# johnviljoen/f16_mpc_oop_py

Hardware: AMD Instinct MI355X
Metric: F16 env steps/sec (hifi Nguyen model, explicit Euler dt=1ms, batch 4096 per GPU) (higher is better)
Workload: dtype f64

## Files before the change

### f16_mpc_oop_py_amd/csrc/f16_dynamics.hip

```cpp
#include <hip/hip_runtime.h>
#include <stdlib.h>

#include <type_traits>

#include "../../include/f16_hip.h"
#include "f16_ctx.h"
#include "f16_plant.hpp"
#include "f16_rollout_common.hpp"
#include "f16_plant_quad.hpp"
#include "f16_mppi.hpp"
#include "f16_gain_sched.hpp"

namespace f16 {

struct CostArgs : SchedArgs {
  const double *x0;
  const double *x_ref;
  const double *u_ref;
  double *x_end;
  long B0, ld0;
  f16_cost_weights w;
};
struct GainSchedArgs : SchedArgs {
  f16_gain_grid grid;
// ... 484 lines not shown
        aero_part<3>((const double *)tab, xa, a.flags, o, sa);
      } else if (wave == 1) {
        aero_part<1>((const double *)tab, xa, a.flags, o, sa);
      } else if (wave == 2) {
        aero_part<2>((const double *)tab, xa, a.flags, o, sa);
      } else {
        double vt = xa[6];
        if (vt <= 0.01) vt = 0.01;
        double mach, qbar, ps;
        atmos_dev(xa[2], vt, mach, qbar, ps);
        xt[12][lane] = qbar; xt[13][lane] = ps;
        aero_part<4>((const double *)tab, xa, a.flags, o, sa);
        if (live) {
          double xq[18];
#pragma unroll
          for (int k = 0; k < 17; ++k) xq[k] = xa[k];
          xq[17] = x[17];
          if (LQR) {
            const double e0 = kq[9] - xa[9], e1 = kq[10] - xa[10], e2 = kq[11] - xa[11];
            double uc[4] = {u[0], 0, 0, 0};
#pragma unroll
            for (int i = 0; i < 3; ++i) ul[i] = uc[1 + i] = lqr_action(kq[3 * i], kq[3 * i + 1], kq[3 * i + 2], e0, e1, e2, u[1 + i]);
            actuators_dev(xq, uc, qbar, ps, xd);
          } else
          actuators_dev(xq, u, qbar, ps, xd);
#pragma unroll
          for (int k = 12; k < 18; ++k) x[k] += xd[k] * a.dt;
        }
        if (tr && --until_store == 0) {
          until_store = a.traj_every;
          if (valid) {
#pragma unroll
            for (int k = 12; k < 18; ++k) __builtin_nontemporal_store(x[k], tr + k * a.ld);
          }
          tr += 18 * a.ld;
        }
        if constexpr (SCHED) if (newrow) {
          ra.take(a, NR, LQR ? kq + 9 : u, a.out + b);
          if (LQR) { ul[0] = u[1]; ul[1] = u[2]; ul[2] = u[3]; }
        }
      }
      const int slot = wave == 1 ? 0 : (wave == 0 ? 3 : (wave == 2 ? 6 : 9));
      xt[slot][lane] = o[0]; xt[slot + 1][lane] = o[1]; xt[slot + 2][lane] = o[2];
      xst[wave][lane] = sa;
      STAMP(tB)
      __syncthreads();
      STAMP(tC)
      if (wave == 0 || wave == 2) {
        double ls[3], ldm[3], ts[3], td[3];
#pragma unroll
        for (int k = 0; k < 3; ++k) { ls[k] = xt[k][lane]; ldm[k] = xt[3 + k][lane]; ts[k] = xt[6 + k][lane]; td[k] = xt[9 + k][lane]; }
        Totals tt;
        compose_totals(ls, ldm, ts, td, a.xcg, tt);
        if (wave == 0) {
          if (live) {
            p.qbar = xt[12][lane]; p.ps = xt[13][lane];
            st |= xst[0][lane] | xst[1][lane] | xst[2][lane] | xst[3][lane];
            plant_forces(xa, p, tt.Cx, tt.Cy, tt.Cz, xd);
#pragma unroll
            for (int k = 0; k < 9; ++k) x[k] += xd[k] * a.dt;
          }
        } else {
          if (live) {
            plant_moments(x[9], x[10], x[11], xt[12][lane], tt.Cl, tt.Cm, tt.Cn, xd);
#pragma unroll
            for (int k = 9; k < 12; ++k) x[k] += xd[k] * a.dt;
          }
          if (tr && --until_store == 0) {
            until_store = a.traj_every;
            if (valid) {
#pragma unroll
              for (int k = 9; k < 12; ++k) __builtin_nontemporal_store(x[k], tr + k * a.ld);
            }
            tr += 18 * a.ld;
          }
        }
      }
    }
#ifdef F16_EXP_STAMP4W
    if (lane == 0 && blockIdx.x == 0 && a.traj) {
      double *d = a.traj + 18 * a.ld * 2 + wave * 4;
      d[0] = (double)tD; d[1] = (double)tA; d[2] = (double)tB; d[3] = (double)tC;
    }
#endif
    if (valid && wave != 1) {
      bool finite = true;
      const int k0 = wave == 0 ? 0 : (wave == 2 ? 9 : 12), k1 = wave == 0 ? 9 : (wave == 2 ? 12 : 18);
#pragma unroll
      for (int k = 0; k < 18; ++k)
        if (k >= k0 && k < k1) { finite = finite && isfinite(x[k]); a.out[k * a.ld + b] = x[k]; }
      if (st & ST_ENVELOPE) st |= envelope_state_bits(x) & (((1 << k1) - (1 << k0)) << 8);
      if (a.status) atomicOr(&a.status[b], st | (finite ? 0 : ST_NONFINITE));
      if (LQR && wave == 3 && a.u_out) {
        a.u_out[b] = u[0];
#pragma unroll
        for (int i = 0; i < 3; ++i) a.u_out[(1 + i) * a.ld + b] = ul[i];
      }
    }
    __syncthreads();
  }
}

template <int GROUPS, bool LQR = false, bool SCHED = false>
__global__ __launch_bounds__(256 * GROUPS) void k_rollout_q(RolloutArgs<SCHED> a) {
  constexpr int NA = 16 * GROUPS;
  constexpr bool G1 = GROUPS == 1;
  __shared__ __attribute__((aligned(16))) double tab[TABLE_IMAGE_DOUBLES];
  __shared__ double xs[18][NA], xt[11][NA];
  __shared__ int xenv[3][NA], xst[2][NA];
  __shared__ double xpsi[3][NA];
#ifdef F16_EXP_STAMPQ
  const unsigned long long tstage0 = __builtin_amdgcn_s_memtime();
#endif
  {
    const double2 *src = reinterpret_cast<const double2 *>(a.tab);
    double2 *dst = reinterpret_cast<double2 *>(tab);
    for (int i = threadIdx.x; i < TABLE_IMAGE_DOUBLES / 2; i += 256 * GROUPS) dst[i] = src[i];
    __syncthreads();
  }
#ifdef F16_EXP_STAMPQ
  const unsigned long long tstage = __builtin_amdgcn_s_memtime() - tstage0;
#endif
  const int role = G1 ? __builtin_amdgcn_readfirstlane((threadIdx.x >> 6) & 3) : (threadIdx.x >> 6) & 3;
  const int grp = threadIdx.x >> 8, lane = threadIdx.x & 63, ac = 16 * grp + (lane >> 2), s = lane & 3;
  const bool envchk = !(a.flags & FLAG_NO_ENVELOPE);
  for (long b0 = (long)blockIdx.x * NA; b0 < a.B; b0 += (long)gridDim.x * NA) {
    const bool valid = b0 + ac < a.B;
    const long b = valid ? b0 + ac : a.B - 1;
    double x[18];
#pragma unroll
    for (int k = 0; k < 18; ++k) x[k] = a.out[k * a.ld + b];
    double ucmd = a.u[s * a.ld + b];
    double kr0 = 0, kr1 = 0, kr2 = 0, dm0 = 0, dm1 = 0, dm2 = 0, ulast = ucmd;
    if (LQR && role == 3) {
      const long row = 9 * (s > 0 ? s - 1 : 0) + 4;
      kr0 = a.K[row * a.ld + b]; kr1 = a.K[(row + 1) * a.ld + b]; kr2 = a.K[(row + 2) * a.ld + b];
      dm0 = a.dem[b]; dm1 = a.dem[a.ld + b]; dm2 = a.dem[2 * a.ld + b];
    }
    double xact = s == 0 ? x[12] : (s == 1 ? x[13] : (s == 2 ? x[14] : x[15]));
    int st = a.status ? a.status[b] : 0;
    double *tr = a.traj ? a.traj + b : nullptr;
    int until_store = a.traj_every;
    QuadCell qc = quad_cell_none();
    LongCorners klong = {};
    LatCorners klat = {};
    RowAhead<1, false> ra;
    double dmq = 0;
    const int rs = LQR && s == 3 ? 2 : s;
    if constexpr (SCHED) {
      dmq = s == 0 ? dm0 : (s == 1 ? dm1 : dm2);
      ra.init(a, LQR ? 3 : 4, a.out + b, rs * a.ld, role == 3);
      ra.settle();
    }
    if (G1 && role == 0 && s == 0) {
      double sp, cp;
      F16_SINCOS_K(reloaded(QUAD_K.sc), x[5], &sp, &cp);
      xpsi[1][ac] = sp; xpsi[2][ac] = cp;
    }
#ifdef F16_EXP_STAMPQ
    unsigned long long tA = 0, tB = 0, tC = 0, tD = 0, t0 = __builtin_amdgcn_s_memtime();
#if F16_EXP_STAMPQ + 0 == 2
#define QSTAMP_WAIT 0xC07F
#else
#define QSTAMP_WAIT 0
#endif
#define QSTAMP(acc) { __builtin_amdgcn_s_waitcnt(QSTAMP_WAIT); unsigned long long t1 = __builtin_amdgcn_s_memtime(); acc += t1 - t0; t0 = t1; }
    unsigned long long tK = 0, tk0 = 0;
#define QK_BEGIN { __builtin_amdgcn_s_waitcnt(QSTAMP_WAIT); tk0 = __builtin_amdgcn_s_memtime(); }
#define QK_END { __builtin_amdgcn_s_waitcnt(QSTAMP_WAIT); tK += __builtin_amdgcn_s_memtime() - tk0; }
#else
#define QSTAMP(acc)
#define QK_BEGIN
#define QK_END
#endif
    if constexpr (G1) {
      switch (role) {
        case 0: {
          constexpr int wave = 0;
#include "f16_quad_steps.inc"
        } break;
        case 1: {
          constexpr int wave = 1;
#include "f16_quad_steps.inc"
        } break;
        case 2: {
          constexpr int wave = 2;
#include "f16_quad_steps.inc"
        } break;
        default: {
          constexpr int wave = 3;
#include "f16_quad_steps.inc"
        } break;
      }
    } else {
      const int wave = role;
#include "f16_quad_steps.inc"
    }
#ifdef F16_EXP_STAMPQ
    if (lane == 0 && blockIdx.x == 0 && a.traj) {
      double *d = a.traj + 18 * a.ld * 2 + role * 4;
      d[0] = (double)tD; d[1] = (double)tA; d[2] = (double)tB; d[3] = (double)tC;
      a.traj[18 * a.ld * 2 + a.ld + role] = (double)tstage;
      a.traj[18 * a.ld * 2 + a.ld + 4 + role] = (double)tK;
    }
#endif
    if (valid) {
      if (role == 2 && s == 0) {
        bool finite = true;
#pragma unroll
        for (int k = 0; k < 9; ++k) { finite = finite && isfinite(x[k]); a.out[k * a.ld + b] = x[k]; }
        if (st & ST_ENVELOPE) st |= envelope_state_bits(x) & (0x1FF << 8);
        if (a.status) atomicOr(&a.status[b], st | (finite ? 0 : ST_NONFINITE));
      } else if (role == 1 && s == 0) {
        bool finite = true;
#pragma unroll
        for (int k = 9; k < 12; ++k) { finite = finite && isfinite(x[k]); a.out[k * a.ld + b] = x[k]; }
        if (st & ST_ENVELOPE) st |= envelope_state_bits(x) & (0x7 << 17);
        if (a.status) atomicOr(&a.status[b], st | (finite ? 0 : ST_NONFINITE));
      } else if (role == 3) {
        a.out[(12 + s) * a.ld + b] = xact;
        bool finite = isfinite(xact);
        if (s < 2) { const double v = s == 0 ? x[16] : x[17]; finite = finite && isfinite(v); a.out[(16 + s) * a.ld + b] = v; }
        if (st & ST_ENVELOPE) {
          const double lim = s == 1 ? 25.0 : (s == 2 ? 21.5 : 30.0);
          if (s == 0 ? (xact < 1000 || xact > 19000) : (xact < -lim || xact > lim)) st |= 1 << (8 + 12 + s);
          if (s == 0 && (x[16] < 0. || x[16] > 25)) st |= 1 << (8 + 16);
        }
        if (a.status) atomicOr(&a.status[b], st | (finite ? 0 : ST_NONFINITE));
        if (LQR && a.u_out) a.u_out[s * a.ld + b] = ulast;
      }
    }
    __syncthreads();
  }
}

struct LinArgsL {
  double *x;
  const double *Ad, *Bd, *K, *xref, *u0;
  double *trx, *tru;
  long B, ld;
  int nsteps, every;
  unsigned track;
};
__global__ __launch_bounds__(64, 1) void k_rollout_lqr_linear(LinArgsL a) {
  const long b = (long)blockIdx.x * 64 + threadIdx.x;
  if (b >= a.B) return;
  double A[81], Bm[27], K[27], x[9], xr[9], u0[3];
#pragma unroll
  for (int e = 0; e < 81; ++e) A[e] = a.Ad[e * a.ld + b];
#pragma unroll
  for (int e = 0; e < 27; ++e) { Bm[e] = a.Bd[e * a.ld + b]; K[e] = a.K[e * a.ld + b]; }
#pragma unroll
  for (int j = 0; j < 9; ++j) { x[j] = a.x[j * a.ld + b]; xr[j] = a.xref[j * a.ld + b]; }
#pragma unroll
  for (int c = 0; c < 3; ++c) u0[c] = a.u0 ? a.u0[c * a.ld + b] : 0.0;
  double *px = a.trx ? a.trx + b : nullptr, *pu = a.tru ? a.tru + b : nullptr;
  int until = a.every;
  for (int t = 0; t < a.nsteps; ++t) {
    double e[9], u[3], xn[9];
#pragma unroll
    for (int j = 0; j < 9; ++j) e[j] = (((a.track >> j) & 1u) ? xr[j] : x[j]) - x[j];
#pragma unroll
    for (int c = 0; c < 3; ++c) {
      double s = 0.0;
#pragma unroll
      for (int j = 0; j < 9; ++j) s += K[9 * c + j] * e[j];
      u[c] = -s + u0[c];
    }
#pragma unroll
    for (int r = 0; r < 9; ++r) {
      double s = 0.0, v = 0.0;
#pragma unroll
      for (int j = 0; j < 9; ++j) s += A[9 * r + j] * x[j];
#pragma unroll
      for (int c = 0; c < 3; ++c) v += Bm[3 * r + c] * u[c];
      xn[r] = s + v;
    }
#pragma unroll
    for (int r = 0; r < 9; ++r) x[r] = xn[r];
    if (--until == 0) {
      until = a.every;
      if (px) {
#pragma unroll
        for (int r = 0; r < 9; ++r) __builtin_nontemporal_store(x[r], px + r * a.ld);
        px += 9 * a.ld;
      }
      if (pu) {
#pragma unroll
        for (int c = 0; c < 3; ++c) __builtin_nontemporal_store(u[c], pu + c * a.ld);
        pu += 3 * a.ld;
      }
    }
  }
#pragma unroll
  for (int r = 0; r < 9; ++r) a.x[r * a.ld + b] = x[r];
}

template <int BLOCK>
__global__ __launch_bounds__(BLOCK) void k_xdot_na(DynArgs a) {
  __shared__ __attribute__((aligned(16))) double tab[TABLE_IMAGE_DOUBLES];
  if (a.fi == 1) stage_tables(tab, a.tab);
  for (long b = (long)blockIdx.x * BLOCK + threadIdx.x; b < a.B; b += (long)gridDim.x * BLOCK) {
    double sv[18], xd9[9];
#pragma unroll
    for (int k = 0; k < 18; ++k) sv[k] = a.x[k * a.ld + b];
    sv[3] = a.u[0 * a.ld + b]; sv[4] = a.u[1 * a.ld + b]; sv[7] = a.u[2 * a.ld + b]; sv[8] = a.u[3 * a.ld + b];
    sv[9] = a.u[4 * a.ld + b]; sv[10] = a.u[5 * a.ld + b]; sv[11] = a.u[6 * a.ld + b];
    sv[17] = a.u[7 * a.ld + b]; sv[16] = a.u[8 * a.ld + b];
    sv[13] = a.u3[0 * a.ld + b]; sv[14] = a.u3[1 * a.ld + b]; sv[15] = a.u3[2 * a.ld + b];
    int st = 0;
    calc_xdot_na((const double *)tab, a.lofi, sv, xd9, a.xcg, a.fi, a.flags, st);
#pragma unroll
    for (int k = 0; k < 9; ++k) a.out[k * a.ld + b] = xd9[k];
    if (a.status) a.status[b] |= st;
  }
}

}

using namespace f16;


extern "C" int f16_xdot_batch(f16_ctx *ctx, const double *x, const double *u, double *xdot, int32_t *status, long B,
                              long ld, double xcg, int fi_flag, unsigned flags, void *stream) {
  if (int rc = check_common(ctx, x, xdot, B, ld)) return rc;
  if (!u) return set_error(F16_EINVAL, "u is NULL");
  if (B == 0) return F16_OK;
  DynArgs a = base_args<DynArgs>(ctx, B, ld, xcg, fi_flag, flags, status);
  a.x = x; a.u = u; a.out = xdot;
  const Geometry g = geometry(B, fi_flag);
  by_block(g, [&](auto block) {
    constexpr int BLOCK = decltype(block)::value;
    if (fi_flag == 0) hipLaunchKernelGGL((k_xdot<BLOCK, 0>), dim3(g.grid), dim3(BLOCK), 0, (hipStream_t)stream, a);
    else hipLaunchKernelGGL((k_xdot<BLOCK, -1>), dim3(g.grid), dim3(BLOCK), 0, (hipStream_t)stream, a);
  });
  return hip_check(hipGetLastError(), "f16_xdot_batch launch");
}

extern "C" int f16_nlplant_batch(f16_ctx *ctx, const double *xu, double *xdot, int32_t *status, long B, long ld,
                                 double xcg, int fi_flag, unsigned flags, void *stream) {
  if (int rc = check_common(ctx, xu, xdot, B, ld)) return rc;
  if (B == 0) return F16_OK;
  DynArgs a = base_args<DynArgs>(ctx, B, ld, xcg, fi_flag, flags, status);
  a.x = xu; a.out = xdot;
  if (B <= 256) {
    hipLaunchKernelGGL((k_nlplant<64, false>), dim3((unsigned)((B + 63) / 64)), dim3(64), 0, (hipStream_t)stream, a);
  } else {
    const Geometry g = geometry(B, fi_flag);
    by_block(g, [&](auto block) {
      constexpr int BLOCK = decltype(block)::value;
      hipLaunchKernelGGL((k_nlplant<BLOCK, true>), dim3(g.grid), dim3(BLOCK), 0, (hipStream_t)stream, a);
    });
  }
  return hip_check(hipGetLastError(), "f16_nlplant_batch launch");
}

// ... 298 lines not shown
```

### f16_mpc_oop_py_amd/csrc/f16_plant.hpp

```cpp
#pragma once
#include <hip/hip_runtime.h>

#include "f16_tables.h"

namespace f16 {

constexpr int ST_ALPHA1 = 1, ST_ALPHA2 = 2, ST_BETA = 4, ST_EL = 8, ST_ENVELOPE = 16, ST_NONFINITE = 32;
constexpr unsigned FLAG_FIX_CLR = 1u, FLAG_NO_ENVELOPE = 2u, FLAG_NO_CELL_CACHE = 16u;

#define F16_DEV __device__ __forceinline__

#ifdef F16_FAST_DIV
#define F16_DIVC(x, c) ((x) * (1.0 / (c)))
#else
#define F16_DIVC(x, c) ((x) / (c))
#endif

__device__ __forceinline__ double f16_rcp(double x) {
#ifdef F16_FAST_DIV
  double r = __builtin_amdgcn_rcp(x);
  r = fma(r, fma(-x, r, 1.0), r);
  r = fma(r, fma(-x, r, 1.0), r);
  return r;
#else
  return 1.0 / x;
#endif
}

struct Axis {
  int j;
  double l;
  double m;
};

F16_DEV double lerp(double f1, double f2, const Axis &a) { return a.l * f2 + a.m * f1; }

F16_DEV double fma_vvs(double a, double b, double c) {
  double d;
  asm("v_fma_f64 %0, %1, %2, %3" : "=v"(d) : "v"(a), "v"(b), "s"(c));
  return d;
}
F16_DEV double fma_svv(double a, double b, double c) {
  double d;
  asm("v_fma_f64 %0, %1, %2, %3" : "=v"(d) : "s"(a), "v"(b), "v"(c));
  return d;
}

struct PowK {
  double log2e, ln2_hi, ln2_lo, nln2_hi, nln2_lo, two_thirds;
  double E[10];
  double L[7];
};
constexpr PowK POW_K = {
    1.44269504088896338700e+00, 6.93147180559945286227e-01, 2.31904681384629955842e-17, -6.93147180559945286227e-01,
    -2.31904681384629955842e-17, 6.66666666666666629659e-01,
    {2.50223225676461415e-08, 2.76309034901126543e-07, 2.75575145458253105e-06, 2.48014910390950412e-05, 1.98412695891155217e-04,
     1.38888889459163820e-03, 8.33333333345504315e-03, 4.16666666665197541e-02, 1.66666666666664770e-01, 5.00000000000001221e-01},
    {1.53670161652585818e-01, 1.52503063567000663e-01, 1.81863527724766383e-01, 2.22221384831011309e-01, 2.85714293974435540e-01,
     3.99999999961319630e-01, 6.66666666666728247e-01}};

F16_DEV double log_k(const PowK &K, double x) {
  const double m = __builtin_amdgcn_frexp_mant(x);
  const bool lo = m < K.two_thirds;
  const double sc = lo ? 2.0 : 1.0;
  const int e = __builtin_amdgcn_frexp_exp(x) + (lo ? -1 : 0);
  const double ym1 = fma(m, sc, -1.0), yp1 = fma(m, sc, 1.0);
  const double ylo = fma(m, sc, -(yp1 + -1.0));
  double r = __builtin_amdgcn_rcp(yp1);
  r = fma(fma(-yp1, r, 1.0), r, r);
  r = fma(fma(-yp1, r, 1.0), r, r);
  const double q = ym1 * r;
  const double p = yp1 * q;
  const double pl = fma(q, ylo, fma(q, yp1, -p));
  const double s25 = fma(yp1, q, pl);
  const double s27 = pl - fma(-yp1, q, s25);
  const double d28 = ym1 - s25;
  const double d32 = d28 + (((ym1 - d28) - s25) - s27);
  const double h = fma(r, d32, q);
  const double l = fma(r, d32, -fma(-ym1, r, h));
  const double z = h * h;
  double c = fma_vvs(z, K.L[0], K.L[1]);
#pragma unroll
  for (int k = 2; k < 7; ++k) c = fma_vvs(z, c, K.L[k]);
  const double a44 = __builtin_ldexp(h, 1), a45 = __builtin_ldexp(l, 1);
  const double t46 = h * z;
  const double u48 = fma(t46, c, a44);
  const double u50 = fma(t46, c, -(u48 - a44));
  const double u51 = a45 + u50;
  const double u52 = u48 + u51;
  const double u54 = u51 - (u52 - u48);
  const double f = (double)e;
  const double g56n = f * K.nln2_hi;
  const double g59 = fma_svv(K.ln2_lo, f, fma_svv(K.ln2_hi, f, g56n));
  const double g60 = fma_svv(K.ln2_hi, f, g59);
  const double g62 = g59 - fma_svv(K.nln2_hi, f, g60);
  const double w63 = g60 + u52;
  const double w64 = w63 - g60;
  const double w68 = (u52 - w64) + (g60 - (w63 - w64));
  const double v69 = g62 + u54;
  const double v70 = v69 - g62;
  const double v74 = (u54 - v70) + (g62 - (v69 - v70));
  const double k75 = v69 + w68;
  const double k76 = w63 + k75;
  const double k80 = k76 + (v74 + (k75 - (k76 - w63)));
  double res = __builtin_fabs(x) == __builtin_inf() ? x : k80;
  res = x < 0.0 ? __builtin_nan("") : res;
  return x == 0.0 ? -__builtin_inf() : res;
}

F16_DEV double exp_k(const PowK &K, double x) {
  const double n = rint(x * K.log2e);
  const double r = fma_svv(K.nln2_lo, n, fma_svv(K.nln2_hi, n, x));
  double c = fma_vvs(r, K.E[0], K.E[1]);
#pragma unroll
  for (int k = 2; k < 10; ++k) c = fma_vvs(r, c, K.E[k]);
  c = fma(r, c, 1.0);
  c = fma(r, c, 1.0);
  double res = __builtin_ldexp(c, (int)n);
  res = x > 1024.0 ? __builtin_inf() : res;
  return x < -1075.0 ? 0.0 : res;
}

template <typename PW>
F16_DEV void atmos_with(double alt, double vt, double &mach, double &qbar, double &ps, PW pw) {
  const double rho0 = 2.377e-3;
  const double tfac = 1 - .703e-5 * alt;
  double temp = 519.0 * tfac;
  if (alt >= 35000.0) temp = 390;
#ifdef F16_FAST_POW
  const double t2 = tfac * tfac;
  const double rho = rho0 * ((t2 * t2) * pw(tfac));
#else
  const double rho = rho0 * pow(tfac, 4.14);
#endif
  mach = vt / sqrt(1.4 * 1716.3 * temp);
  qbar = .5 * rho * (vt * vt);
  ps = 1715.0 * rho * temp;
  if (ps == 0) ps = 1715;
}
F16_DEV void atmos_dev(double alt, double vt, double &mach, double &qbar, double &ps) {
  atmos_with(alt, vt, mach, qbar, ps, [](double tfac) { return exp(0.14 * log(tfac)); });
}
F16_DEV void atmos_dev_k(const PowK &K, double alt, double vt, double &mach, double &qbar, double &ps) {
  atmos_with(alt, vt, mach, qbar, ps, [&K](double tfac) { return exp_k(K, 0.14 * log_k(K, tfac)); });
}


struct SinCosK {
  double two_over_pi, npio2[3];
  double S[8], C[9];
};
constexpr SinCosK SINCOS_K = {
    6.36619772367581382433e-01, {-1.57079632673412561417e+00, -6.07710050630396597660e-11, -2.02226624879595063154e-21},
    {-1.66666666666666657e-01, 8.33333333333333322e-03, -1.98412698412698413e-04, 2.75573192239858925e-06, -2.50521083854417202e-08, 1.60590438368216133e-10, -7.64716373181981641e-13, 2.81145725434552060e-15},
    {-5.00000000000000000e-01, 4.16666666666666644e-02, -1.38888888888888894e-03, 2.48015873015873016e-05, -2.75573192239858883e-07, 2.08767569878681002e-09, -1.14707455977297245e-11, 4.77947733238738525e-14, -1.56192069685862253e-16}};

struct QuadK { SinCosK sc; PowK pw; };
static __constant__ const QuadK QUAD_K = {SINCOS_K, POW_K};
template <typename T>
F16_DEV T reloaded(const T &t) {
  static_assert(sizeof(T) % sizeof(double) == 0, "a table of doubles");
  unsigned long p = reinterpret_cast<unsigned long>(&t);
  asm volatile("" : "+s"(p));
  const __attribute__((address_space(4))) double *q = (const __attribute__((address_space(4))) double *)p;
  T k;
  double *d = reinterpret_cast<double *>(&k);
#pragma unroll
  for (unsigned i = 0; i < sizeof(T) / sizeof(double); ++i) d[i] = q[i];
  return k;
}

#ifdef F16_FAST_TRIG
F16_DEV void sincos_quadrant(double n, double s0, double c0, double *sn, double *cs) {
  const int k = (int)n & 3;
  const double a = (k & 1) ? c0 : s0, b = (k & 1) ? s0 : c0;
  *sn = (k & 2) ? -a : a;
  *cs = ((k + 1) & 2) ? -b : b;
}

F16_DEV void sincos_bf(double x, double *sn, double *cs) {
  constexpr SinCosK K = SINCOS_K;
  const double n = rint(x * K.two_over_pi);
  double r = fma(-n, -K.npio2[0], x);
  r = fma(-n, -K.npio2[1], r);
  r = fma(-n, -K.npio2[2], r);
  const double z = r * r;
  double p = K.S[7], q = K.C[8];
#pragma unroll
  for (int k = 6; k >= 0; --k) p = fma(p, z, K.S[k]);
#pragma unroll
  for (int k = 7; k >= 0; --k) q = fma(q, z, K.C[k]);
  const double s0 = fma(r * z, p, r), c0 = fma(z, q, 1.0);
  sincos_quadrant(n, s0, c0, sn, cs);
}

F16_DEV void sincos_bf_k(const SinCosK &K, double x, double *sn, double *cs) {
  const double n = rint(x * K.two_over_pi);
  double r = fma_svv(K.npio2[0], n, x);
  r = fma_svv(K.npio2[1], n, r);
  r = fma_svv(K.npio2[2], n, r);
  const double z = r * r;
  double p = K.S[7], q = K.C[8];
#pragma unroll
  for (int k = 6; k >= 0; --k) p = fma_vvs(p, z, K.S[k]);
#pragma unroll
  for (int k = 7; k >= 0; --k) q = fma_vvs(q, z, K.C[k]);
  const double s0 = fma(r * z, p, r), c0 = fma(z, q, 1.0);
  sincos_quadrant(n, s0, c0, sn, cs);
}
#define F16_SINCOS(x, s, c) sincos_bf(x, s, c)
#define F16_SINCOS_K(K, x, s, c) sincos_bf_k(K, x, s, c)
#else
#define F16_SINCOS(x, s, c) sincos(x, s, c)
#define F16_SINCOS_K(K, x, s, c) sincos(x, s, c)
#endif

struct Aero {
  double Cx, Cz, Cm, Cy, Cn, Cl;
  double Cxq, Cyr, Cyp, Czq, Clr, Clp, Cmq, Cnr, Cnp;
  double dCx_lef, dCz_lef, dCm_lef, dCy_lef, dCn_lef, dCl_lef;
  double dCxq_lef, dCyr_lef, dCyp_lef, dCzq_lef, dClr_lef, dClp_lef, dCmq_lef, dCnr_lef, dCnp_lef;
  double dCy_r30, dCn_r30, dCl_r30;
  double dCy_a20, dCy_a20_lef, dCn_a20, dCn_a20_lef, dCl_a20, dCl_a20_lef;
  double dCnbeta, dClbeta, dCm, eta_el;
};

struct BrRaw { double lo, hi, xm, xg, xg1, xp; int g; };
template <typename TP>
F16_DEV BrRaw br_load(TP X, int n, int guess) {
  BrRaw r;
  r.g = min(max(guess, 0), n - 2);
  r.lo = X[0]; r.hi = X[n - 1];
  r.xm = X[max(r.g - 1, 0)]; r.xg = X[r.g]; r.xg1 = X[r.g + 1]; r.xp = X[min(r.g + 2, n - 1)];
  return r;
}
struct BrCell { int j; double v, x0, x1; };
F16_DEV BrCell br_cell(const BrRaw &r, int n, double v, bool &off) {
  off = !(v >= r.lo && v <= r.hi);
  v = fmin(fmax(v, r.lo), r.hi);
  const bool down = r.g > 0 && v < r.xg, up = r.g < n - 2 && v >= r.xg1;
  BrCell c;
  c.j = r.g - (down ? 1 : 0) + (up ? 1 : 0);
  c.v = v;
  c.x0 = down ? r.xm : (up ? r.xg1 : r.xg);
  c.x1 = down ? r.xg : (up ? r.xp : r.xg1);
  return c;
}
F16_DEV Axis br_axis(const BrCell &c) {
  Axis a;
  a.j = c.j;
#ifdef F16_FAST_DIV
  a.l = c.v == c.x1 ? 1.0 : (c.v - c.x0) * f16_rcp(c.x1 - c.x0);
#else
  a.l = (c.v - c.x0) / (c.x1 - c.x0);
#endif
  a.m = 1 - a.l;
  return a;
}
struct Q4 { double f00, f10, f01, f11; };
template <typename TP>
F16_DEV Q4 ld4(TP p, int sa, int sb) { Q4 c; c.f00 = p[0]; c.f10 = p[sa]; c.f01 = p[sb]; c.f11 = p[sb + sa]; return c; }
F16_DEV double bil4(const Q4 &c, const Axis &a, const Axis &b) {
  return lerp(lerp(c.f00, c.f10, a), lerp(c.f01, c.f11, a), b);
}
struct W4 { double w00, w10, w01, w11; };
F16_DEV W4 bil_weights(const Axis &a, const Axis &b) { W4 w; w.w00 = a.m * b.m; w.w10 = a.l * b.m; w.w01 = a.m * b.l; w.w11 = a.l * b.l; return w; }
#ifdef F16_FAST_DIV
F16_DEV double bil4w(const Q4 &c, const Axis &, const Axis &, const W4 &w) { return w.w00 * c.f00 + w.w10 * c.f10 + w.w01 * c.f01 + w.w11 * c.f11; }
#else
F16_DEV double bil4w(const Q4 &c, const Axis &a, const Axis &b, const W4 &) { return bil4(c, a, b); }
#endif
#ifndef F16_PHASE_MASK
#define F16_PHASE_MASK 0x7
#endif
#define F16_PHASE() __builtin_amdgcn_sched_barrier(F16_PHASE_MASK)

F16_DEV int alpha_guess(double alpha) { return (int)((fmin(fmax(alpha, -20.0), 90.0) + 20.0) * 0.2); }
F16_DEV int beta_guess(double beta) {
  const double bc = fmin(fmax(beta, -30.0), 30.0);
  return bc < -10.0 ? (int)((bc + 30.0) * 0.2) : (bc < 10.0 ? 4 + (int)((bc + 10.0) * 0.5) : 14 + (int)((bc - 10.0) * 0.2));
}


struct TotalsOut { double Cx, Cz, Cm, Cy, Cn, Cl; };

struct TabI32 { const int *base; };
struct I32View {
  const int *p;
  F16_DEV I32View operator+(int o) const { return I32View{p + o}; }
  F16_DEV double operator[](int i) const { return (double)p[i]; }
};
template <typename TP> struct Lay {
  static constexpr int G3A = OFF_G3A, SG3A = S_G3A, G3B = OFF_G3B, SG3B = S_G3B, G2A = OFF_G2A, SG2A = S_G2A, G2B = OFF_G2B,
                       SG2B = S_G2B, G1A = OFF_G1A, SG1A = S_G1A, G1B = OFF_G1B, SG1B = S_G1B, ETA = OFF_ETA;
  static constexpr bool SCALED = false;
  static F16_DEV TP tab(TP T) { return T; }
  static F16_DEV TP bp(TP T) { return T; }
};
template <> struct Lay<TabI32> {
  static constexpr int G3A = i32::OFF_G3A, SG3A = i32::S_G3A, G3B = i32::OFF_G3B, SG3B = i32::S_G3B, G2A = i32::OFF_G2A,
                       SG2A = i32::S_G2A, G2B = i32::OFF_G2B, SG2B = i32::S_G2B, G1A = i32::OFF_G1A, SG1A = i32::S_G1A,
                       G1B = i32::OFF_G1B, SG1B = i32::S_G1B, ETA = i32::OFF_ETA;
  static constexpr bool SCALED = true;
  static F16_DEV I32View tab(TabI32 T) { return I32View{T.base}; }
  static F16_DEV const double *bp(TabI32 T) { return reinterpret_cast<const double *>(T.base); }
};

template <typename TP>
F16_DEV void aero_totals_phased(TP T0, const double *xu, double xcg, unsigned flags, TotalsOut &t, int &status) {
  using L = Lay<TP>;
  const auto T = L::tab(T0);
  const auto BP = L::bp(T0);
  constexpr int S_G3A = L::SG3A, S_G3B = L::SG3B, S_G2A = L::SG2A, S_G2B = L::SG2B, S_G1A = L::SG1A, S_G1B = L::SG1B;
  constexpr int OFF_G3A = L::G3A, OFF_G3B = L::G3B, OFF_G2A = L::G2A, OFF_G2B = L::G2B, OFF_G1A = L::G1A, OFF_G1B = L::G1B,
                OFF_ETA = L::ETA;
  const double B = 30.0, cbar = 11.32, xcgr = 0.35, r2d = 180.0 / 3.141592653589793;
  double vt = xu[6];
  if (vt <= 0.01) vt = 0.01;
  const double alpha = xu[7] * r2d, beta = xu[8] * r2d, P = xu[9], Q = xu[10], R = xu[11], el = xu[13];
  const double dail = F16_DIVC(xu[14], 21.5), drud = F16_DIVC(xu[15], 30.0), dlef = 1 - F16_DIVC(xu[16], 25.0);
  const double r2vt = f16_rcp(2 * vt), kq = cbar * r2vt, kb = B * r2vt;
  const BrRaw ra = br_load(BP + OFF_BP_A1, N_A1, alpha_guess(alpha));
  const BrRaw rb = br_load(BP + OFF_BP_B1, N_B1, beta_guess(beta));
  const BrRaw r1 = br_load(BP + OFF_BP_D1, N_D1, (el >= -10.0) + (el >= 0.0) + (el >= 10.0));
  const BrRaw r2 = br_load(BP + OFF_BP_D2, N_D2, (int)(el >= 0.0));
  const double a45 = BP[OFF_BP_A1 + N_A2 - 1];
  F16_PHASE();
  bool offa, offb, off1, off2;
  const BrCell ca = br_cell(ra, N_A1, alpha, offa), cb = br_cell(rb, N_B1, beta, offb);
  const BrCell c1 = br_cell(r1, N_D1, el, off1), c2 = br_cell(r2, N_D2, el, off2);
  if (offa) status |= ST_ALPHA1 | ST_ALPHA2;
  if (offb) status |= ST_BETA;
  if (off1) status |= ST_EL;
  const bool hi_a = ca.j > N_A2 - 2;
  if (hi_a && alpha > a45) status |= ST_ALPHA2;
  const int j2 = hi_a ? N_A2 - 2 : ca.j;
  const int n1 = cb.j * N_A1 + ca.j, n2 = cb.j * N_A2 + j2;
  const Axis a1 = br_axis(ca), b = br_axis(cb), d1 = br_axis(c1), d2 = br_axis(c2);
  Axis a2 = a1;
  if (hi_a) { a2.j = N_A2 - 2; a2.l = 1.0; a2.m = 0.0; }
  const auto g = T + OFF_G1A + ca.j * S_G1A, h = T + OFF_G1B + j2 * S_G1B;
  {
    constexpr int SA = S_G3A, SB = S_G3A * N_A1, SD = S_G3A * N_A1 * N_B1;
    const auto p = T + OFF_G3A + n1 * SA;
    Q4 qlo[3], qhi[3], q0[3], ql[3];
    double g0[3], g1[3], h0[3], h1[3];
#pragma unroll
    for (int k = 0; k < 3; ++k) {
      qlo[k] = ld4(p + k + c1.j * SD, SA, SB); qhi[k] = ld4(p + k + (c1.j + 1) * SD, SA, SB);
      q0[k] = ld4(p + k + D1_ZERO_NODE * SD, SA, SB);
      ql[k] = ld4(T + OFF_G2B + n2 * S_G2B + k, S_G2B, S_G2B * N_A2);
      g0[k] = g[3 * k]; g1[k] = g[S_G1A + 3 * k]; h0[k] = h[3 * k]; h1[k] = h[S_G1B + 3 * k];
    }
    const double m0 = g[11], m1 = g[S_G1A + 11], e0 = T[OFF_ETA + c1.j], e1 = T[OFF_ETA + c1.j + 1];
    F16_PHASE();
    const W4 W1 = bil_weights(a1, b);
    double Cf[3], dC[3], dQ[3];
#pragma unroll
    for (int k = 0; k < 3; ++k) {
      Cf[k] = lerp(bil4w(qlo[k], a1, b, W1), bil4w(qhi[k], a1, b, W1), d1);
      dC[k] = bil4(ql[k], a2, b) - bil4w(q0[k], a1, b, W1);
      const double Cq = lerp(g0[k], g1[k], a1), dq = lerp(h0[k], h1[k], a2);
      dQ[k] = kq * (Cq + (k == 1 ? dC[k] : dq) * dlef);
    }
    t.Cx = Cf[0] + dC[0] * dlef + dQ[0] * Q;
// ... 644 lines not shown
```

### f16_mpc_oop_py_amd/csrc/f16_quad_steps.inc

```
    for (int t = 0; t <= a.nsteps; ++t) {
      if (wave == 2) {
        xenv[0][ac] = envchk && (x[2] < 0 || x[2] > 100000 || x[6] < 0 || x[6] > 900 || x[7] < -20. || x[7] > 90 ||
                                 x[8] < -30. || x[8] > 30);
        if (s == 0) {
#pragma unroll
          for (int k = 0; k < 9; ++k) xs[k][ac] = x[k];
        }
      } else if (wave == 1) {
        xenv[1][ac] = envchk && (x[9] < -300 || x[9] > 300 || x[10] < -100 || x[10] > 100 || x[11] < -50 || x[11] > 50);
        if (s < 3) xs[9 + s][ac] = s == 0 ? x[9] : (s == 1 ? x[10] : x[11]);
      } else if (wave == 3) {
        const double lim = s == 1 ? 25.0 : (s == 2 ? 21.5 : 30.0);
        const bool bad = s == 0 ? (xact < 1000 || xact > 19000) : (xact < -lim || xact > lim);
        const bool badl = x[16] < 0. || x[16] > 25;
        if (s == 0) xenv[2][ac] = 0;
        xs[12 + s][ac] = xact;
        if (s < 2) xs[16 + s][ac] = s == 0 ? x[16] : x[17];
        __builtin_amdgcn_wave_barrier();
        if (envchk && (bad || badl)) xenv[2][ac] = 1;
      }
      QSTAMP(tD)
      __syncthreads();
      QSTAMP(tA)
      double xa[17];
      int env_any = 0;
      if constexpr (G1) {
        env_any = xenv[0][ac] | xenv[1][ac] | xenv[2][ac];
#pragma unroll
        for (int k = 0; k < 17; ++k) xa[k] = xs[k][ac];
      }
      if (wave == 2 && tr && t > 0 && --until_store == 0) {
        until_store = a.traj_every;
        if (valid) {
          if constexpr (G1) {
            double smp[5];
#pragma unroll
            for (int j = 0; j < 5; ++j) smp[j] = xs[s + 4 * j < 18 ? s + 4 * j : s][ac];
            __builtin_amdgcn_sched_barrier(0);
#pragma unroll
            for (int j = 0; j < 5; ++j) {
              const int kk = s + 4 * j;
              if (kk < 18) __builtin_nontemporal_store(smp[j], tr + kk * a.ld);
            }
          } else {
#pragma unroll
            for (int j = 0; j < 5; ++j) {
              const int kk = s + 4 * j;
              if (kk < 18) __builtin_nontemporal_store(xs[kk][ac], tr + kk * a.ld);
            }
          }
        }
        tr += 18 * a.ld;
      }
      if (t == a.nsteps) break;
      if constexpr (!G1) {
        env_any = xenv[0][ac] | xenv[1][ac] | xenv[2][ac];
#pragma unroll
        for (int k = 0; k < 17; ++k) xa[k] = xs[k][ac];
      }
      if ((!G1 || wave != 0) && env_any) st |= ST_ENVELOPE;
      const bool live = !(st & ST_ENVELOPE);
      double xd[9] = {0, 0, 0, 0, 0, 0, 0, 0, 0};
      double U = 0, V = 0, W = 0, s_t = 0, c_t = 0, s_phi = 0, c_phi = 0, cb = 0, vtc = 0, r1 = 0, r2 = 0, r3 = 0;
      double fu0 = 0, fv0 = 0, fw0 = 0, mo0 = 0, mo1 = 0, mo2 = 0;
      bool newrow = false;
      if constexpr (SCHED) newrow = ra.due(a, LQR ? 3 : 4);
      if (wave == 0) {
        int sa_ = 0;
        double latd;
        const double tot = quad_long<G1>((const double *)tab, xa, s, a.xcg, a.flags, qc, klong, latd, sa_);
        if (s < 3) { xt[s][ac] = tot; xt[8 + s][ac] = latd; }
        xst[0][ac] = sa_;
      } else if (wave == 1) {
        int sa_ = 0;
        const double tot = quad_lat<G1>((const double *)tab, xa, s, a.flags, qc, klat, sa_);
        if (s < 3) xt[3 + s][ac] = tot;
        xst[1][ac] = sa_;
        {
          const double Jy = 55814.0, Jxz = 982.0, Jz = 63100.0, Jx = 9496.0;
          const double rden = 1.0 / (9496.0 * 63100.0 - 982.0 * 982.0);
          const double P = x[9], Q = x[10], R = x[11];
          mo0 = (Jxz * (Jx - Jy + Jz) * P * Q - (Jz * (Jz - Jy) + Jxz * Jxz) * Q * R) * rden;
          mo1 = F16_DIVC((Jz - Jx) * P * R - Jxz * (P * P - R * R), Jy);
          mo2 = ((Jx * (Jx - Jy) + Jxz * Jxz) * P * Q - Jxz * (Jx - Jy + Jz) * Q * R) * rden;
        }
        if constexpr (G1) quad_taken_here(mo0, mo1, mo2);
      } else if (wave == 2) {
        const double ang = s == 0 ? xa[3] : (s == 1 ? xa[4] : (s == 2 ? (G1 ? xa[8] : xa[5]) : xa[7]));
        double sn, cs, sb, s_psi, c_psi;
        if constexpr (G1) {
          QK_BEGIN
          const auto ksc = reloaded(QUAD_K.sc);
          QK_END
          F16_SINCOS_K(ksc, ang, &sn, &cs);
        } else F16_SINCOS(ang, &sn, &cs);
        if constexpr (G1) { sb = quad_bcast<2>(sn); cb = quad_bcast<2>(cs); } else F16_SINCOS(xa[8], &sb, &cb);
        s_phi = quad_bcast<0>(sn); c_phi = quad_bcast<0>(cs);
        s_t = quad_bcast<1>(sn); c_t = quad_bcast<1>(cs);
        if constexpr (G1) { s_psi = xpsi[1][ac]; c_psi = xpsi[2][ac]; } else { s_psi = quad_bcast<2>(sn); c_psi = quad_bcast<2>(cs); }
        const double sal = quad_bcast<3>(sn), cal = quad_bcast<3>(cs);
        vtc = xa[6];
        if (vtc <= 0.01) vtc = 0.01;
        U = vtc * cal * cb; V = vtc * sb; W = vtc * sal * cb;
        const double P = xa[9], Q = xa[10], R = xa[11];
#ifdef F16_FAST_DIV
        const double rct = f16_rcp(c_t);
        const double tt = s_t * rct;
#elif defined(F16_FAST_TAN)
        const double rct = 0.0, tt = s_t / c_t;
#else
        const double rct = 0.0, tt = tan(xa[4]);
#endif
        xd[0] = U * (c_t * c_psi) + V * (s_phi * c_psi * s_t - c_phi * s_psi) + W * (c_phi * s_t * c_psi + s_phi * s_psi);
        xd[1] = U * (c_t * s_psi) + V * (s_phi * s_psi * s_t + c_phi * c_psi) + W * (c_phi * s_t * s_psi - s_phi * c_psi);
        xd[2] = U * s_t - V * (s_phi * c_t) - W * (c_phi * c_t);
        xd[3] = P + tt * (Q * s_phi + R * c_phi);
        xd[4] = Q * c_phi - R * s_phi;
#ifdef F16_FAST_DIV
        xd[5] = (Q * s_phi + R * c_phi) * rct;
        r1 = f16_rcp(vtc); r2 = f16_rcp(U * U + W * W); r3 = f16_rcp(vtc * vtc * cb);
#else
        xd[5] = (Q * s_phi + R * c_phi) / c_t;
        (void)rct;
#endif
        {
          const double g = 32.17, m = 636.94;
          fu0 = R * V - Q * W - g * s_t + F16_DIVC(xa[12], m);
          fv0 = P * W - R * U + g * c_t * s_phi;
          fw0 = Q * U - P * V + g * c_t * c_phi;
          if (live) {
#pragma unroll
            for (int k = 0; k < 6; ++k) x[k] += xd[k] * a.dt;
          }
          if (G1 && s == 0) xpsi[0][ac] = x[5];
        }
        if constexpr (G1) quad_taken_here(U, V, W, vtc, r1, r2, r3, fu0, fv0, fw0);
      } else {
        double vt = xa[6];
        if (vt <= 0.01) vt = 0.01;
        double mach, qbar, ps;
        double pw = 0;
        if constexpr (G1) {
          QK_BEGIN
          const PowK pk = reloaded(QUAD_K.pw);
          QK_END
          atmos_with(xa[2], vt, mach, qbar, ps, [&](double tfac) { return pw = exp_k(pk, 0.14 * log_k(pk, tfac)); });
        } else
          atmos_dev(xa[2], vt, mach, qbar, ps);
        if (s == 0) { xt[6][ac] = qbar; xt[7][ac] = ps; }
        if (live) {
          const double lim = s == 1 ? 25.0 : (s == 2 ? 21.5 : 30.0), rate = s == 1 ? 60.0 : (s == 2 ? 80.0 : 120.0);
          double uc = ucmd;
          if (LQR) {
            if constexpr (SCHED) { dm0 = quad_bcast<0>(dmq); dm1 = quad_bcast<1>(dmq); dm2 = quad_bcast<2>(dmq); }
            const double ua = lqr_action(kr0, kr1, kr2, dm0 - xa[9], dm1 - xa[10], dm2 - xa[11], ucmd);
            uc = s > 0 ? ua : ucmd;
            ulast = uc;
          }
          const double dth = actuator_rate(ucmd, 1000, 19000, 1.0, xact, 10000);
          const double dsf = actuator_rate(uc, -lim, lim, 20.2, xact, rate);
          double lf1_dot, lf2_dot;
          if constexpr (G1)
            upd_lef_with(xa[2], xa[6], xa[7], x[17], x[16], qbar, ps, lf1_dot, lf2_dot,
                         [pw](double h_, double V_, double &m_, double &q_, double &p_) {
                           atmos_with(h_, V_, m_, q_, p_, [pw](double) { return pw; });
                         });
          else
            upd_lef_dev(xa[2], xa[6], xa[7], x[17], x[16], qbar, ps, lf1_dot, lf2_dot);
          xact += (s == 0 ? dth : dsf) * a.dt;
          x[16] += lf2_dot * a.dt;
          x[17] += lf1_dot * a.dt;
        }
        if constexpr (SCHED) if (newrow) {
          int rv;
          asm volatile("v_mbcnt_lo_u32_b32 %0, -1, 0\n\tv_mbcnt_hi_u32_b32 %0, -1, %0" : "=v"(rv));
          rv &= 3;
          if (LQR && rv == 3) rv = 2;
          ra.take(a, LQR ? 3 : 4, LQR ? &dmq : &ucmd, a.out + b, rv * a.ld);
          if (LQR) ulast = ucmd;
        }
      }
      QSTAMP(tB)
      __syncthreads();
      QSTAMP(tC)
      if (wave == 2) {
        if (live) {
          st |= xst[0][ac] | xst[1][ac];
          const double Cx = xt[0][ac], Cz = xt[1][ac], Cy = xt[3][ac] + xt[8][ac], qbar = xt[6][ac];
          const double m = 636.94, S = 300.0;
          const double qsm = F16_DIVC(qbar * S, m);
          const double Udot = fu0 + qsm * Cx;
          const double Vdot = fv0 + qsm * Cy;
          const double Wdot = fw0 + qsm * Cz;
#ifdef F16_FAST_DIV
          xd[6] = (U * Udot + V * Vdot + W * Wdot) * r1;
          xd[7] = (U * Wdot - W * Udot) * r2;
          xd[8] = (Vdot * vtc - V * xd[6]) * r3;
#else
          xd[6] = (U * Udot + V * Vdot + W * Wdot) / vtc;
          xd[7] = (U * Wdot - W * Udot) / (U * U + W * W);
          xd[8] = (Vdot * vtc - V * xd[6]) / (vtc * vtc * cb);
#endif
#pragma unroll
          for (int k = 6; k < 9; ++k) x[k] += xd[k] * a.dt;
        }
      } else if (wave == 1) {
        if (live) {
          const double Cy = xt[3][ac] + xt[8][ac];
          const double Cn = xt[4][ac] + xt[9][ac] - Cy * (0.35 - a.xcg) * (11.32 / 30.0);
          const double Cl = xt[5][ac] + xt[10][ac];
          const double Jy = 55814.0, Jxz = 982.0, Jz = 63100.0, Jx = 9496.0, S = 300.0;
          const double rden = 1.0 / (9496.0 * 63100.0 - 982.0 * 982.0);
          const double qs = xt[6][ac] * S;
          const double L_tot = Cl * qs * 30.0, M_tot = xt[2][ac] * qs * 11.32, N_tot = Cn * qs * 30.0;
          x[9] += (mo0 + (Jz * L_tot + Jxz * N_tot) * rden) * a.dt;
          x[10] += (mo1 + F16_DIVC(M_tot, Jy)) * a.dt;
          x[11] += (mo2 + (Jx * N_tot + Jxz * L_tot) * rden) * a.dt;
        }
      } else if (G1 && wave == 0 && s == 0) {
        double sp, cp;
        QK_BEGIN
        const auto ksc = reloaded(QUAD_K.sc);
        QK_END
        F16_SINCOS_K(ksc, xpsi[0][ac], &sp, &cp);
        xpsi[1][ac] = sp; xpsi[2][ac] = cp;
      }
    }
```

Measured before the change: 4.487 billion.

## Hoist constant tables out of step loop, pin in VGPRs, trim per-wave state

Loads the sincos and pow polynomial coefficient tables once per wave before the time-step loop instead of reloading them every step. Wave 2 keeps its table in VGPRs through a templated FMA variant that uses vector operands. Unowned state entries are zeroed per wave so they drop out of registers. Envelope altitude checks and xs stores are moved into the post-barrier phase and LDS reads are hoisted ahead of a sched_barrier. This trades more register pressure for fewer scalar loads and a shorter critical path per step, and adds scheduling complexity.

```diff
diff --git a/f16_mpc_oop_py_amd/csrc/f16_dynamics.hip b/f16_mpc_oop_py_amd/csrc/f16_dynamics.hip
--- a/f16_mpc_oop_py_amd/csrc/f16_dynamics.hip
+++ b/f16_mpc_oop_py_amd/csrc/f16_dynamics.hip
@@ -660,11 +660,6 @@
       ra.init(a, LQR ? 3 : 4, a.out + b, rs * a.ld, role == 3);
       ra.settle();
     }
-    if (G1 && role == 0 && s == 0) {
-      double sp, cp;
-      F16_SINCOS_K(reloaded(QUAD_K.sc), x[5], &sp, &cp);
-      xpsi[1][ac] = sp; xpsi[2][ac] = cp;
-    }
 #ifdef F16_EXP_STAMPQ
     unsigned long long tA = 0, tB = 0, tC = 0, tD = 0, t0 = __builtin_amdgcn_s_memtime();
 #if F16_EXP_STAMPQ + 0 == 2
@@ -673,13 +668,8 @@
 #define QSTAMP_WAIT 0
 #endif
 #define QSTAMP(acc) { __builtin_amdgcn_s_waitcnt(QSTAMP_WAIT); unsigned long long t1 = __builtin_amdgcn_s_memtime(); acc += t1 - t0; t0 = t1; }
-    unsigned long long tK = 0, tk0 = 0;
-#define QK_BEGIN { __builtin_amdgcn_s_waitcnt(QSTAMP_WAIT); tk0 = __builtin_amdgcn_s_memtime(); }
-#define QK_END { __builtin_amdgcn_s_waitcnt(QSTAMP_WAIT); tK += __builtin_amdgcn_s_memtime() - tk0; }
 #else
 #define QSTAMP(acc)
-#define QK_BEGIN
-#define QK_END
 #endif
     if constexpr (G1) {
       switch (role) {
@@ -709,7 +699,6 @@
       double *d = a.traj + 18 * a.ld * 2 + role * 4;
       d[0] = (double)tD; d[1] = (double)tA; d[2] = (double)tB; d[3] = (double)tC;
       a.traj[18 * a.ld * 2 + a.ld + role] = (double)tstage;
-      a.traj[18 * a.ld * 2 + a.ld + 4 + role] = (double)tK;
     }
 #endif
     if (valid) {
diff --git a/f16_mpc_oop_py_amd/csrc/f16_plant.hpp b/f16_mpc_oop_py_amd/csrc/f16_plant.hpp
--- a/f16_mpc_oop_py_amd/csrc/f16_plant.hpp
+++ b/f16_mpc_oop_py_amd/csrc/f16_plant.hpp
@@ -44,6 +44,26 @@
   double d;
   asm("v_fma_f64 %0, %1, %2, %3" : "=v"(d) : "s"(a), "v"(b), "v"(c));
   return d;
+}
+F16_DEV double fma_vvv(double a, double b, double c) {
+  double d;
+  asm("v_fma_f64 %0, %1, %2, %3" : "=v"(d) : "v"(a), "v"(b), "v"(c));
+  return d;
+}
+struct KScalar {
+  static F16_DEV double vvk(double a, double b, double k) { return fma_vvs(a, b, k); }
+  static F16_DEV double kvv(double k, double b, double c) { return fma_svv(k, b, c); }
+};
+struct KVector {
+  static F16_DEV double vvk(double a, double b, double k) { return fma_vvv(a, b, k); }
+  static F16_DEV double kvv(double k, double b, double c) { return fma_vvv(k, b, c); }
+};
+F16_DEV void in_vgpr(double &x) { asm volatile("" : "+v"(x)); }
+template <typename T>
+F16_DEV void table_in_vgprs(T &t) {
+  double *d = reinterpret_cast<double *>(&t);
+#pragma unroll
+  for (unsigned i = 0; i < sizeof(T) / sizeof(double); ++i) in_vgpr(d[i]);
 }
 
 struct PowK {
@@ -59,6 +79,7 @@
     {1.53670161652585818e-01, 1.52503063567000663e-01, 1.81863527724766383e-01, 2.22221384831011309e-01, 2.85714293974435540e-01,
      3.99999999961319630e-01, 6.66666666666728247e-01}};
 
+template <typename OP = KScalar>
 F16_DEV double log_k(const PowK &K, double x) {
   const double m = __builtin_amdgcn_frexp_mant(x);
   const bool lo = m < K.two_thirds;
@@ -79,9 +100,9 @@
   const double h = fma(r, d32, q);
   const double l = fma(r, d32, -fma(-ym1, r, h));
   const double z = h * h;
-  double c = fma_vvs(z, K.L[0], K.L[1]);
-#pragma unroll
-  for (int k = 2; k < 7; ++k) c = fma_vvs(z, c, K.L[k]);
+  double c = OP::vvk(z, K.L[0], K.L[1]);
+#pragma unroll
+  for (int k = 2; k < 7; ++k) c = OP::vvk(z, c, K.L[k]);
   const double a44 = __builtin_ldexp(h, 1), a45 = __builtin_ldexp(l, 1);
   const double t46 = h * z;
   const double u48 = fma(t46, c, a44);
@@ -91,9 +112,9 @@
   const double u54 = u51 - (u52 - u48);
   const double f = (double)e;
   const double g56n = f * K.nln2_hi;
-  const double g59 = fma_svv(K.ln2_lo, f, fma_svv(K.ln2_hi, f, g56n));
-  const double g60 = fma_svv(K.ln2_hi, f, g59);
-  const double g62 = g59 - fma_svv(K.nln2_hi, f, g60);
+  const double g59 = OP::kvv(K.ln2_lo, f, OP::kvv(K.ln2_hi, f, g56n));
+  const double g60 = OP::kvv(K.ln2_hi, f, g59);
+  const double g62 = g59 - OP::kvv(K.nln2_hi, f, g60);
   const double w63 = g60 + u52;
   const double w64 = w63 - g60;
   const double w68 = (u52 - w64) + (g60 - (w63 - w64));
@@ -108,12 +129,13 @@
   return x == 0.0 ? -__builtin_inf() : res;
 }
 
+template <typename OP = KScalar>
 F16_DEV double exp_k(const PowK &K, double x) {
   const double n = rint(x * K.log2e);
-  const double r = fma_svv(K.nln2_lo, n, fma_svv(K.nln2_hi, n, x));
-  double c = fma_vvs(r, K.E[0], K.E[1]);
-#pragma unroll
-  for (int k = 2; k < 10; ++k) c = fma_vvs(r, c, K.E[k]);
+  const double r = OP::kvv(K.nln2_lo, n, OP::kvv(K.nln2_hi, n, x));
+  double c = OP::vvk(r, K.E[0], K.E[1]);
+#pragma unroll
+  for (int k = 2; k < 10; ++k) c = OP::vvk(r, c, K.E[k]);
   c = fma(r, c, 1.0);
   c = fma(r, c, 1.0);
   double res = __builtin_ldexp(c, (int)n);
@@ -194,23 +216,26 @@
   sincos_quadrant(n, s0, c0, sn, cs);
 }
 
+template <typename OP = KScalar>
 F16_DEV void sincos_bf_k(const SinCosK &K, double x, double *sn, double *cs) {
   const double n = rint(x * K.two_over_pi);
-  double r = fma_svv(K.npio2[0], n, x);
-  r = fma_svv(K.npio2[1], n, r);
-  r = fma_svv(K.npio2[2], n, r);
+  double r = OP::kvv(K.npio2[0], n, x);
+  r = OP::kvv(K.npio2[1], n, r);
+  r = OP::kvv(K.npio2[2], n, r);
   const double z = r * r;
   double p = K.S[7], q = K.C[8];
 #pragma unroll
-  for (int k = 6; k >= 0; --k) p = fma_vvs(p, z, K.S[k]);
-#pragma unroll
-  for (int k = 7; k >= 0; --k) q = fma_vvs(q, z, K.C[k]);
+  for (int k = 6; k >= 0; --k) p = OP::vvk(p, z, K.S[k]);
+#pragma unroll
+  for (int k = 7; k >= 0; --k) q = OP::vvk(q, z, K.C[k]);
   const double s0 = fma(r * z, p, r), c0 = fma(z, q, 1.0);
   sincos_quadrant(n, s0, c0, sn, cs);
 }
 #define F16_SINCOS(x, s, c) sincos_bf(x, s, c)
 #define F16_SINCOS_K(K, x, s, c) sincos_bf_k(K, x, s, c)
+#define F16_SINCOS_KC(OP, K, x, s, c) sincos_bf_k<OP>(K, x, s, c)
 #else
+#define F16_SINCOS_KC(OP, K, x, s, c) sincos(x, s, c)
 #define F16_SINCOS(x, s, c) sincos(x, s, c)
 #define F16_SINCOS_K(K, x, s, c) sincos(x, s, c)
 #endif
diff --git a/f16_mpc_oop_py_amd/csrc/f16_quad_steps.inc b/f16_mpc_oop_py_amd/csrc/f16_quad_steps.inc
--- a/f16_mpc_oop_py_amd/csrc/f16_quad_steps.inc
+++ b/f16_mpc_oop_py_amd/csrc/f16_quad_steps.inc
@@ -1,10 +1,42 @@
+    [[maybe_unused]] SinCosK ksc = {};
+    [[maybe_unused]] PowK kpw = {};
+    [[maybe_unused]] bool env_h = false;
+    if constexpr (G1) {
+      if (wave == 0 || wave == 2) ksc = reloaded(QUAD_K.sc);
+      if (wave == 3) kpw = reloaded(QUAD_K.pw);
+      if (wave == 2) table_in_vgprs(ksc);
+      if (wave == 0) { in_vgpr(ksc.S[7]); in_vgpr(ksc.C[8]); }
+      if (wave == 3) { in_vgpr(kpw.E[0]); in_vgpr(kpw.L[0]); }
+      if (wave == 0 && s == 0) {
+        double sp, cp;
+        F16_SINCOS_K(ksc, x[5], &sp, &cp);
+        xpsi[1][ac] = sp; xpsi[2][ac] = cp;
+      }
+      if (wave == 2) {
+        env_h = envchk && (x[2] < 0 || x[2] > 100000);
+        if (s == 0) {
+#pragma unroll
+          for (int k = 0; k < 6; ++k) xs[k][ac] = x[k];
+        }
+      }
+      if (wave != 3) {
+#pragma unroll
+        for (int k = 0; k < 18; ++k)
+          if (!(wave == 2 ? k < 9 : (wave == 1 && k >= 9 && k < 12))) x[k] = 0;
+      }
+    }
     for (int t = 0; t <= a.nsteps; ++t) {
       if (wave == 2) {
-        xenv[0][ac] = envchk && (x[2] < 0 || x[2] > 100000 || x[6] < 0 || x[6] > 900 || x[7] < -20. || x[7] > 90 ||
-                                 x[8] < -30. || x[8] > 30);
-        if (s == 0) {
-#pragma unroll
-          for (int k = 0; k < 9; ++k) xs[k][ac] = x[k];
+        if constexpr (G1) {
+          xenv[0][ac] = env_h | (envchk & ((x[6] < 0) | (x[6] > 900) | (x[7] < -20.) | (x[7] > 90) | (x[8] < -30.) | (x[8] > 30)));
+          xs[6 + (s < 3 ? s : 2)][ac] = s == 0 ? x[6] : (s == 1 ? x[7] : x[8]);
+        } else {
+          xenv[0][ac] = envchk && (x[2] < 0 || x[2] > 100000 || x[6] < 0 || x[6] > 900 || x[7] < -20. || x[7] > 90 ||
+                                   x[8] < -30. || x[8] > 30);
+          if (s == 0) {
+#pragma unroll
+            for (int k = 0; k < 9; ++k) xs[k][ac] = x[k];
+          }
         }
       } else if (wave == 1) {
         xenv[1][ac] = envchk && (x[9] < -300 || x[9] > 300 || x[10] < -100 || x[10] > 100 || x[11] < -50 || x[11] > 50);
@@ -88,12 +120,8 @@
       } else if (wave == 2) {
         const double ang = s == 0 ? xa[3] : (s == 1 ? xa[4] : (s == 2 ? (G1 ? xa[8] : xa[5]) : xa[7]));
         double sn, cs, sb, s_psi, c_psi;
-        if constexpr (G1) {
-          QK_BEGIN
-          const auto ksc = reloaded(QUAD_K.sc);
-          QK_END
-          F16_SINCOS_K(ksc, ang, &sn, &cs);
-        } else F16_SINCOS(ang, &sn, &cs);
+        if constexpr (G1) F16_SINCOS_KC(KVector, ksc, ang, &sn, &cs);
+        else F16_SINCOS(ang, &sn, &cs);
         if constexpr (G1) { sb = quad_bcast<2>(sn); cb = quad_bcast<2>(cs); } else F16_SINCOS(xa[8], &sb, &cb);
         s_phi = quad_bcast<0>(sn); c_phi = quad_bcast<0>(cs);
         s_t = quad_bcast<1>(sn); c_t = quad_bcast<1>(cs);
@@ -140,12 +168,9 @@
         if (vt <= 0.01) vt = 0.01;
         double mach, qbar, ps;
         double pw = 0;
-        if constexpr (G1) {
-          QK_BEGIN
-          const PowK pk = reloaded(QUAD_K.pw);
-          QK_END
-          atmos_with(xa[2], vt, mach, qbar, ps, [&](double tfac) { return pw = exp_k(pk, 0.14 * log_k(pk, tfac)); });
-        } else
+        if constexpr (G1)
+          atmos_with(xa[2], vt, mach, qbar, ps, [&](double tfac) { return pw = exp_k(kpw, 0.14 * log_k(kpw, tfac)); });
+        else
           atmos_dev(xa[2], vt, mach, qbar, ps);
         if (s == 0) { xt[6][ac] = qbar; xt[7][ac] = ps; }
         if (live) {
@@ -184,9 +209,22 @@
       __syncthreads();
       QSTAMP(tC)
       if (wave == 2) {
+        int sx = 0;
+        double t0_ = 0, t1_ = 0, t3_ = 0, t8_ = 0, t6_ = 0;
+        if constexpr (G1) {
+          sx = xst[0][ac] | xst[1][ac];
+          t0_ = xt[0][ac]; t1_ = xt[1][ac]; t3_ = xt[3][ac]; t8_ = xt[8][ac]; t6_ = xt[6][ac];
+          __builtin_amdgcn_sched_barrier(0);
+          env_h = envchk & ((x[2] < 0) | (x[2] > 100000));
+          if (s == 0) {
+#pragma unroll
+            for (int k = 0; k < 6; ++k) xs[k][ac] = x[k];
+          }
+        }
         if (live) {
-          st |= xst[0][ac] | xst[1][ac];
-          const double Cx = xt[0][ac], Cz = xt[1][ac], Cy = xt[3][ac] + xt[8][ac], qbar = xt[6][ac];
+          if constexpr (!G1) { sx = xst[0][ac] | xst[1][ac]; t0_ = xt[0][ac]; t1_ = xt[1][ac]; t3_ = xt[3][ac]; t8_ = xt[8][ac]; t6_ = xt[6][ac]; }
+          st |= sx;
+          const double Cx = t0_, Cz = t1_, Cy = t3_ + t8_, qbar = t6_;
           const double m = 636.94, S = 300.0;
           const double qsm = F16_DIVC(qbar * S, m);
           const double Udot = fu0 + qsm * Cx;
@@ -219,9 +257,6 @@
         }
       } else if (G1 && wave == 0 && s == 0) {
         double sp, cp;
-        QK_BEGIN
-        const auto ksc = reloaded(QUAD_K.sc);
-        QK_END
         F16_SINCOS_K(ksc, xpsi[0][ac], &sp, &cp);
         xpsi[1][ac] = sp; xpsi[2][ac] = cp;
       }
```

Result: faster. 4.612 billion, median of 6 (+2.8%).
